# LukasHaas/PIGEON

Measured on AMD Instinct MI355X. Metric: images/sec end-to-end (ViT+head+refine), 4x336x336, higher is better.
Workload: dtype f16

## Files before the change

### pigeon_amd/csrc/head.hip

```cpp
#include "common.h"
#include "pigeon_internal.h"
#include "certainty_common.h"
#include <cfloat>

#define HT 64
#define HK 32

__global__ __launch_bounds__(256) void head_logits_kernel(const float* __restrict__ emb, int B, int P,
                                                          const float* __restrict__ W, const float* __restrict__ bias,
                                                          int C, float* __restrict__ logits) {
    __shared__ float As[HK][HT + 1];
    __shared__ float Ws[HK][HT + 1];
    const int tid = threadIdx.x;
    const int c0 = blockIdx.x * HT, b0 = blockIdx.y * HT;
    const int tx = tid & 15, ty = tid >> 4;
    float acc[4][4];
#pragma unroll
    for (int i = 0; i < 4; ++i)
#pragma unroll
        for (int j = 0; j < 4; ++j) acc[i][j] = 0.f;
    const float invP = 1.0f / (float)P;
    for (int k0 = 0; k0 < VIT_HIDDEN; k0 += HK) {
#pragma unroll
        for (int i = 0; i < 8; ++i) {
            const int idx = tid + i * 256;
            const int r = idx >> 5, k = idx & 31;
            float a = 0.f;
            if (b0 + r < B) {
                const float* e = emb + ((int64_t)(b0 + r) * P) * VIT_HIDDEN + k0 + k;
                for (int p = 0; p < P; ++p) a += e[(int64_t)p * VIT_HIDDEN];
                a *= invP;
            }
            As[k][r] = a;
            Ws[k][r] = (c0 + r < C) ? W[(int64_t)(c0 + r) * VIT_HIDDEN + k0 + k] : 0.f;
        }
        __syncthreads();
#pragma unroll
        for (int k = 0; k < HK; ++k) {
            float a[4], w[4];
#pragma unroll
            for (int i = 0; i < 4; ++i) a[i] = As[k][ty * 4 + i];
#pragma unroll
            for (int j = 0; j < 4; ++j) w[j] = Ws[k][tx * 4 + j];
#pragma unroll
            for (int i = 0; i < 4; ++i)
#pragma unroll
                for (int j = 0; j < 4; ++j) acc[i][j] = fmaf(a[i], w[j], acc[i][j]);
        }
        __syncthreads();
    }
#pragma unroll
    for (int i = 0; i < 4; ++i) {
        const int b = b0 + ty * 4 + i;
        if (b >= B) continue;
#pragma unroll
        for (int j = 0; j < 4; ++j) {
            const int c = c0 + tx * 4 + j;
            if (c < C) logits[(int64_t)b * C + c] = acc[i][j] + bias[c];
        }
    }
}

struct ValIdx { float v; int i; };
__device__ __forceinline__ ValIdx block_argbest(ValIdx x, ValIdx* red ) {
#pragma unroll
    for (int o = 32; o >= 1; o >>= 1) {
        const float ov = __shfl_xor(x.v, o, 64);
        const int oi = __shfl_xor(x.i, o, 64);
        if (better(ov, oi, x.v, x.i)) { x.v = ov; x.i = oi; }
    }
    const int wave = threadIdx.x >> 6;
    __syncthreads();
    if ((threadIdx.x & 63) == 0) red[wave] = x;
    __syncthreads();
    ValIdx r = red[0];
#pragma unroll
    for (int w = 1; w < 4; ++w) if (better(red[w].v, red[w].i, r.v, r.i)) r = red[w];
    return r;
}

template <bool GLOBAL>
__global__ __launch_bounds__(256) void head_row_kernel(const float* __restrict__ logits, int C, int k,
                                                       const double* __restrict__ centroids,
                                                       float* __restrict__ topk_val, int64_t* __restrict__ topk_idx,
                                                       int64_t* __restrict__ argmax_out, double* __restrict__ pred_llh,
                                                       float* __restrict__ scratch) {
    extern __shared__ __attribute__((aligned(16))) float probs_lds[];
    float* probs = GLOBAL ? scratch + (int64_t)blockIdx.x * C : probs_lds;
    __shared__ ValIdx red[4];
    __shared__ float redf[4];
    const int b = blockIdx.x, tid = threadIdx.x;
    const float* row = logits + (int64_t)b * C;
    float mx = -FLT_MAX;
    for (int c = tid; c < C; c += 256) { const float v = row[c]; probs[c] = v; mx = fmaxf(mx, v); }
    mx = wave_max(mx);
    if ((tid & 63) == 0) redf[tid >> 6] = mx;
    __syncthreads();
    mx = fmaxf(fmaxf(redf[0], redf[1]), fmaxf(redf[2], redf[3]));
    __syncthreads();
    float sm = 0.f;
    for (int c = tid; c < C; c += 256) { const float e = expf(probs[c] - mx); probs[c] = e; sm += e; }
    sm = wave_sum(sm);
    if ((tid & 63) == 0) redf[tid >> 6] = sm;
    __syncthreads();
    sm = (redf[0] + redf[1]) + (redf[2] + redf[3]);
    for (int c = tid; c < C; c += 256) probs[c] = probs[c] / sm;
    __syncthreads();
    for (int r = 0; r < k; ++r) {
        ValIdx best; best.v = -1.f; best.i = 0x7fffffff;
        for (int c = tid; c < C; c += 256) {
            const float v = probs[c];
            if (better(v, c, best.v, best.i)) { best.v = v; best.i = c; }
        }
        best = block_argbest(best, red);
        if (tid == 0) {
            if (best.i < 0 || best.i >= C) best.i = r < C ? r : C - 1;
            topk_val[(int64_t)b * k + r] = best.v;
            topk_idx[(int64_t)b * k + r] = best.i;
            if (r == 0) {
                argmax_out[b] = best.i;
                pred_llh[2 * b] = centroids[2 * (int64_t)best.i];
                pred_llh[2 * b + 1] = centroids[2 * (int64_t)best.i + 1];
            }
            probs[best.i] = -2.f;
        }
        if (GLOBAL) __threadfence_block();
        __syncthreads();
    }
}

extern "C" int pg_head_forward(const float* emb, int B, int P, const float* W, const float* bias,
                               const double* centroids, int C, int k, float* logits, float* topk_val,
                               int64_t* topk_idx, int64_t* argmax, double* pred_llh, void* stream) {
    hipStream_t s = (hipStream_t)stream;
    if (B < 0) { pg_set_error("head: B = %d", B); return PG_EINVAL; }
    if (B == 0) return PG_OK;
    if (!emb || !W || !bias || !centroids || !logits || !topk_val || !topk_idx || !argmax || !pred_llh) {
        pg_set_error("head: null pointer argument"); return PG_EINVAL;
    }
    if (P < 1 || C < 1 || k < 1 || k > C) { pg_set_error("head: bad P=%d C=%d k=%d", P, C, k); return PG_EINVAL; }
    const size_t lds = (size_t)C * sizeof(float);
    const bool big = lds > 150 * 1024;
    dim3 g1((C + HT - 1) / HT, (B + HT - 1) / HT);
    hipLaunchKernelGGL(head_logits_kernel, g1, dim3(256), 0, s, emb, B, P, W, bias, C, logits);
    int rc = pg_check_launch("head_logits");
    if (rc) return rc;
    if (big) {
        float* scratch = nullptr;
        PG_HIP(hipMallocAsync((void**)&scratch, (size_t)B * C * sizeof(float), s));
        hipLaunchKernelGGL(head_row_kernel<true>, dim3(B), dim3(256), 0, s, logits, C, k, centroids, topk_val, topk_idx, argmax, pred_llh, scratch);
        rc = pg_check_launch("head_row (large C)");
        (void)hipFreeAsync(scratch, s);
        return rc;
    }
    static size_t attr_lds = 0;
    if (lds > attr_lds) {
        PG_HIP(hipFuncSetAttribute((const void*)head_row_kernel<false>, hipFuncAttributeMaxDynamicSharedMemorySize, (int)lds));
        attr_lds = lds;
    }
    hipLaunchKernelGGL(head_row_kernel<false>, dim3(B), dim3(256), lds, s, logits, C, k, centroids, topk_val, topk_idx, argmax, pred_llh,
                       (float*)nullptr);
    return pg_check_launch("head_row");
}

__global__ __launch_bounds__(256) void head_margin_kernel(const float* __restrict__ logits, int C, const float* __restrict__ emb, int P,
                                                          const float* __restrict__ W, float* __restrict__ margin,
                                                          float* __restrict__ sens, int64_t* __restrict__ top2) {
    __shared__ ValIdx red[4];
    __shared__ float redf[8];
    const int b = blockIdx.x, tid = threadIdx.x;
    const float* row = logits + (int64_t)b * C;
    ValIdx b1; b1.v = -FLT_MAX; b1.i = 0x7fffffff;
    bool any = false;
    for (int c = tid; c < C; c += 256) { const float v = row[c]; if (!any || better(v, c, b1.v, b1.i)) { b1.v = v; b1.i = c; any = true; } }
    if (!any) { b1.v = -FLT_MAX; b1.i = 0x7fffffff; }
    const ValIdx t1 = block_argbest(b1, red);
    ValIdx b2; b2.v = -FLT_MAX; b2.i = 0x7fffffff;
    any = false;
    for (int c = tid; c < C; c += 256) {
        if (c == t1.i) continue;
        const float v = row[c];
        if (!any || better(v, c, b2.v, b2.i)) { b2.v = v; b2.i = c; any = true; }
    }
    if (!any) { b2.v = -FLT_MAX; b2.i = 0x7fffffff; }
    __syncthreads();
    const ValIdx t2 = block_argbest(b2, red);
    const bool have2 = C > 1 && t2.i >= 0 && t2.i < C;
    float se = 0.f, sw = 0.f;
    {
        const int c0 = tid * 4;
        const float invP = 1.0f / (float)P;
#pragma unroll
        for (int e = 0; e < 4; ++e) {
            float a = 0.f;
            for (int p = 0; p < P; ++p) a += emb[((int64_t)b * P + p) * VIT_HIDDEN + c0 + e];
            a *= invP;
            se += a * a;
            if (have2) { const float d = W[(int64_t)t1.i * VIT_HIDDEN + c0 + e] - W[(int64_t)t2.i * VIT_HIDDEN + c0 + e]; sw += d * d; }
        }
    }
    se = wave_sum(se); sw = wave_sum(sw);
    __syncthreads();
    if ((tid & 63) == 0) { redf[tid >> 6] = se; redf[4 + (tid >> 6)] = sw; }
    __syncthreads();
    if (tid == 0) {
        se = (redf[0] + redf[1]) + (redf[2] + redf[3]);
        sw = (redf[4] + redf[5]) + (redf[6] + redf[7]);
        margin[b] = have2 ? t1.v - t2.v : INFINITY;
        sens[b] = have2 ? sqrtf(se) * sqrtf(sw) * (1.0f / 32.0f) : 0.f;
        if (top2) top2[b] = have2 ? t2.i : t1.i;
    }
}

extern "C" int pg_head_margin(const float* logits, int B, int C, const float* emb, int P, const float* W, float* margin, float* sens,
                              int64_t* top2, void* stream) {
    if (B < 0) { pg_set_error("head_margin: B = %d", B); return PG_EINVAL; }
    if (B == 0) return PG_OK;
    if (!logits || !emb || !W || !margin || !sens) { pg_set_error("head_margin: null pointer argument"); return PG_EINVAL; }
    if (P < 1 || C < 1) { pg_set_error("head_margin: bad P=%d C=%d", P, C); return PG_EINVAL; }
    hipLaunchKernelGGL(head_margin_kernel, dim3(B), dim3(256), 0, (hipStream_t)stream, logits, C, emb, P, W, margin, sens, top2);
    return pg_check_launch("head_margin");
}
```

Before: 2452.

## Split head into mean-pool kernel and skinny-B GEMV-style logits kernel

Moves the patch mean-pooling into its own kernel that writes an interleaved per-row-group layout, so pooling is no longer recomputed by every column block of the logits GEMM. The logits kernel becomes a small-batch GEMV design: each wave handles NB rows across 64 columns, W slabs are double-buffered in LDS with register prefetch, and blocks are swizzled across the 8 XCDs. This targets the old 64x64 tile that wasted most of its work on B=4 and re-read embeddings per column tile. It adds an extra launch and a per-call async malloc/free of the pooled buffer.

Measured after the change: 2457 (median of 6 runs). No clear change (+0.2%).

```diff
diff --git a/pigeon_amd/csrc/head.hip b/pigeon_amd/csrc/head.hip
--- a/pigeon_amd/csrc/head.hip
+++ b/pigeon_amd/csrc/head.hip
@@ -3,62 +3,94 @@
 #include "certainty_common.h"
 #include <cfloat>
 
-#define HT 64
+#define HC 64
 #define HK 32
-
-__global__ __launch_bounds__(256) void head_logits_kernel(const float* __restrict__ emb, int B, int P,
-                                                          const float* __restrict__ W, const float* __restrict__ bias,
-                                                          int C, float* __restrict__ logits) {
-    __shared__ float As[HK][HT + 1];
-    __shared__ float Ws[HK][HT + 1];
-    const int tid = threadIdx.x;
-    const int c0 = blockIdx.x * HT, b0 = blockIdx.y * HT;
-    const int tx = tid & 15, ty = tid >> 4;
-    float acc[4][4];
-#pragma unroll
-    for (int i = 0; i < 4; ++i)
-#pragma unroll
-        for (int j = 0; j < 4; ++j) acc[i][j] = 0.f;
-    const float invP = 1.0f / (float)P;
-    for (int k0 = 0; k0 < VIT_HIDDEN; k0 += HK) {
-#pragma unroll
-        for (int i = 0; i < 8; ++i) {
-            const int idx = tid + i * 256;
-            const int r = idx >> 5, k = idx & 31;
-            float a = 0.f;
-            if (b0 + r < B) {
-                const float* e = emb + ((int64_t)(b0 + r) * P) * VIT_HIDDEN + k0 + k;
-                for (int p = 0; p < P; ++p) a += e[(int64_t)p * VIT_HIDDEN];
-                a *= invP;
+#define HLD (HK + 4)
+
+__global__ __launch_bounds__(256) void head_mean_kernel(const float* __restrict__ emb, int B, int B_pad, int P, int nb,
+                                                        float* __restrict__ am) {
+    const int64_t i = (int64_t)blockIdx.x * 256 + threadIdx.x;
+    if (i >= (int64_t)B_pad * VIT_HIDDEN) return;
+    const int64_t b = i / VIT_HIDDEN, k = i % VIT_HIDDEN;
+    float a = 0.f;
+    if (b < B) {
+        const float* e = emb + b * P * VIT_HIDDEN + k;
+        for (int p = 0; p < P; ++p) a += e[(int64_t)p * VIT_HIDDEN];
+        a *= 1.0f / (float)P;
+    }
+    am[((b / nb) * VIT_HIDDEN + k) * nb + b % nb] = a;
+}
+
+template <int NB>
+__global__ __launch_bounds__(256) void head_logits_kernel(const float* __restrict__ am, int B, const float* __restrict__ W,
+                                                          const float* __restrict__ bias, int C, int row_groups,
+                                                          float* __restrict__ logits) {
+    __shared__ __attribute__((aligned(16))) float Ws[2][HC * HLD];
+    const int tid = threadIdx.x, lane = tid & 63;
+    const int wave = __builtin_amdgcn_readfirstlane(tid >> 6);
+    const int xcd = blockIdx.x & 7, slot = blockIdx.x >> 3;
+    const int cb = (slot / row_groups) * 8 + xcd;
+    if (cb * HC >= C) return;
+    const int c0 = cb * HC;
+    const int r0 = ((slot % row_groups) * 4 + wave) * NB;
+    const bool active = r0 < B;
+    const int sr = tid >> 3, sk = (tid & 7) * 4;
+    const float* wsrc[2];
+#pragma unroll
+    for (int i = 0; i < 2; ++i) {
+        const int c = c0 + sr + 32 * i;
+        wsrc[i] = W + (int64_t)(c < C ? c : C - 1) * VIT_HIDDEN + sk;
+    }
+    const float* arow = am + (int64_t)r0 * VIT_HIDDEN;
+    float acc[NB];
+#pragma unroll
+    for (int r = 0; r < NB; ++r) acc[r] = 0.f;
+
+    float4 wl0 = *(const float4*)wsrc[0], wl1 = *(const float4*)wsrc[1];
+    float* wdst = &Ws[0][sr * HLD + sk];
+    *(float4*)wdst = wl0;
+    *(float4*)(wdst + 32 * HLD) = wl1;
+    __syncthreads();
+    constexpr int NSLAB = VIT_HIDDEN / HK;
+    for (int s = 0; s < NSLAB; ++s) {
+        const int k0 = s * HK;
+        if (s + 1 < NSLAB) {
+            wl0 = *(const float4*)(wsrc[0] + k0 + HK);
+            wl1 = *(const float4*)(wsrc[1] + k0 + HK);
+        }
+        if (active) {
+            const float* ws = &Ws[s & 1][lane * HLD];
+#pragma unroll
+            for (int kc = 0; kc < HK; kc += 4) {
+                const float4 w4 = *(const float4*)(ws + kc);
+                const float w[4] = {w4.x, w4.y, w4.z, w4.w};
+#pragma unroll
+                for (int r = 0; r < NB; ++r) {
+                    const float* a = arow + (k0 + kc) * NB + r;
+#pragma unroll
+                    for (int j = 0; j < 4; ++j) acc[r] = fmaf(a[j * NB], w[j], acc[r]);
+                }
             }
-            As[k][r] = a;
-            Ws[k][r] = (c0 + r < C) ? W[(int64_t)(c0 + r) * VIT_HIDDEN + k0 + k] : 0.f;
+        }
+        if (s + 1 < NSLAB) {
+            float* d = wdst + ((s + 1) & 1) * (HC * HLD);
+            *(float4*)d = wl0;
+            *(float4*)(d + 32 * HLD) = wl1;
         }
         __syncthreads();
-#pragma unroll
-        for (int k = 0; k < HK; ++k) {
-            float a[4], w[4];
-#pragma unroll
-            for (int i = 0; i < 4; ++i) a[i] = As[k][ty * 4 + i];
-#pragma unroll
-            for (int j = 0; j < 4; ++j) w[j] = Ws[k][tx * 4 + j];
-#pragma unroll
-            for (int i = 0; i < 4; ++i)
-#pragma unroll
-                for (int j = 0; j < 4; ++j) acc[i][j] = fmaf(a[i], w[j], acc[i][j]);
-        }
-        __syncthreads();
-    }
-#pragma unroll
-    for (int i = 0; i < 4; ++i) {
-        const int b = b0 + ty * 4 + i;
-        if (b >= B) continue;
-#pragma unroll
-        for (int j = 0; j < 4; ++j) {
-            const int c = c0 + tx * 4 + j;
-            if (c < C) logits[(int64_t)b * C + c] = acc[i][j] + bias[c];
-        }
-    }
+    }
+    const int c = c0 + lane;
+    if (!active || c >= C) return;
+    const float bc = bias[c];
+#pragma unroll
+    for (int r = 0; r < NB; ++r)
+        if (r0 + r < B) logits[(int64_t)(r0 + r) * C + c] = acc[r] + bc;
+}
+
+template <int NB>
+static void head_logits_launch(const float* am, int B, const float* W, const float* bias, int C, float* logits, hipStream_t s) {
+    const int col_blocks = ((C + HC - 1) / HC + 7) / 8 * 8, row_groups = (B + 4 * NB - 1) / (4 * NB);
+    hipLaunchKernelGGL(head_logits_kernel<NB>, dim3(col_blocks * row_groups), dim3(256), 0, s, am, B, W, bias, C, row_groups, logits);
 }
 
 struct ValIdx { float v; int i; };
@@ -141,9 +173,20 @@
     if (P < 1 || C < 1 || k < 1 || k > C) { pg_set_error("head: bad P=%d C=%d k=%d", P, C, k); return PG_EINVAL; }
     const size_t lds = (size_t)C * sizeof(float);
     const bool big = lds > 150 * 1024;
-    dim3 g1((C + HT - 1) / HT, (B + HT - 1) / HT);
-    hipLaunchKernelGGL(head_logits_kernel, g1, dim3(256), 0, s, emb, B, P, W, bias, C, logits);
-    int rc = pg_check_launch("head_logits");
+    const int nb = B <= 4 ? 1 : B <= 8 ? 2 : B <= 16 ? 4 : 8;
+    const int B_pad = (B + 4 * nb - 1) / (4 * nb) * (4 * nb);
+    float* am = nullptr;
+    PG_HIP(hipMallocAsync((void**)&am, (size_t)B_pad * VIT_HIDDEN * sizeof(float), s));
+    hipLaunchKernelGGL(head_mean_kernel, dim3((unsigned)(((int64_t)B_pad * VIT_HIDDEN + 255) / 256)), dim3(256), 0, s, emb, B, B_pad, P, nb, am);
+    int rc = pg_check_launch("head_mean");
+    if (!rc) {
+        if (nb == 1) head_logits_launch<1>(am, B, W, bias, C, logits, s);
+        else if (nb == 2) head_logits_launch<2>(am, B, W, bias, C, logits, s);
+        else if (nb == 4) head_logits_launch<4>(am, B, W, bias, C, logits, s);
+        else head_logits_launch<8>(am, B, W, bias, C, logits, s);
+        rc = pg_check_launch("head_logits");
+    }
+    (void)hipFreeAsync(am, s);
     if (rc) return rc;
     if (big) {
         float* scratch = nullptr;
```
